# ImNotPrepared/Dynamic3DGaussians

Hardware: AMD Instinct MI355X
Metric: rendered Mpix/s fwd+bwd (1/8 GPU) at 300k Gaussians; PSNR vs ref (higher is better)
Workload: dtype f32

## Files before the change

dynamic3dgaussians_amd/csrc/gs_api.hip:

```cpp
#include <stdarg.h>
#include <stdio.h>
#include <stdlib.h>
#include <string.h>

#include <mutex>
#include <string>
#include <thread>
#include <vector>

#include "../../include/gs_camera_grad.h"
#include "../../include/gs_track.h"
#include "../../include/gs_window.h"
#include "../../include/gsplat_hip.h"
#include "gs_common.h"
#include "gs_kernels.h"
#include "gs_launch.h"

using namespace gs;

namespace {
#define fail gs_set_error

int higher_msb(uint32_t n) {
  uint32_t msb = sizeof(n) * 4, step = msb;
// ... 92 lines not shown
};
thread_local PlanInfo g_plan;

struct HeaderSlot {
  uint32_t* host = nullptr;
  uint32_t* dev = nullptr;
  int device = -1;
};
std::mutex g_hmu;
std::vector<HeaderSlot> g_hfree;

struct HeaderLease {
  HeaderSlot s;
  bool in_flight = false;
  hipStream_t stream = nullptr;
  void launched(hipStream_t s_) {
    in_flight = true;
    stream = s_;
  }
  HeaderLease() {
    int device = 0;
    if (hipGetDevice(&device) != hipSuccess) return;
    {
      std::lock_guard<std::mutex> lk(g_hmu);
      for (size_t i = g_hfree.size(); i-- > 0;) {
        if (g_hfree[i].device != device) continue;
        s = g_hfree[i];
        g_hfree.erase(g_hfree.begin() + (std::ptrdiff_t)i);
        return;
      }
    }
    s.device = device;
    void* h = nullptr;
    if (hipHostMalloc(&h, sizeof(uint32_t) * GS_MAX_CAMS * M_WORDS,
                      hipHostMallocMapped | hipHostMallocCoherent) != hipSuccess)
      return;
    void* d = nullptr;
    if (hipHostGetDevicePointer(&d, h, 0) != hipSuccess) {
      (void)hipHostFree(h);
      s = HeaderSlot{};
      return;
    }
    s.host = static_cast<uint32_t*>(h);
    s.dev = static_cast<uint32_t*>(d);
  }
  ~HeaderLease() {
    if (!s.host) return;
    if (in_flight && hipStreamSynchronize(stream) != hipSuccess) return;
    std::lock_guard<std::mutex> lk(g_hmu);
    g_hfree.push_back(s);
  }
  bool ok() const { return s.host != nullptr; }
};

struct SortPlan {
  int64_t max_len = -1;
  int64_t total = -1;
  SortClasses sc;
  bool hinted = false;
};

SortCover sort_cover(const SortPlan& sp, int64_t tiles) {
  SortCover cv;
  if (sp.max_len < 0 || !sp.sc.valid || !sp.hinted) return cv;
  cv.on = 1;
  cv.q1 = sp.sc.q1;
  cv.p1 = sp.sc.p1;
  cv.p2 = sp.sc.p2;
  cv.mid = sp.max_len > SORT_SMALL;
  cv.lng = sp.max_len > TS_CAP;
  (void)tiles;
  return cv;
}

TileArgs tile_args(int P, int W, int H, void* geom, void* image, const int32_t* walk = nullptr) {
  TileArgs t{};
  t.walk = walk;
  const GeomLayout gl(P);
  const ImgLayout il(W, H);
  t.P = P; t.W = W; t.H = H;
  t.grid_x = (W + TILE - 1) / TILE; t.grid_y = (H + TILE - 1) / TILE;
  t.num_tiles = (int)il.tiles;
  t.rect = at<uint4>(geom, gl.rect);
  t.tiles = at<uint32_t>(geom, gl.tiles);
  t.rec = at<float>(geom, gl.rec);
  t.thist = at<uint32_t>(image, il.thist);
  t.ttotal = at<uint32_t>(image, il.ttotal);
  t.bsum = at<uint32_t>(image, il.bsum);
  t.meta = at<uint32_t>(image, il.meta);
  t.ranges = at<uint2>(image, il.ranges);
  t.order = at<uint4>(image, il.order);
  t.fmax = at<uint32_t>(image, il.fmax);
  return t;
}
}

extern "C" {

int gs_timing_enable(int enable) {
  std::lock_guard<std::mutex> lk(g_tmu);
  for (auto& e : g_events) { g_pool.push_back(e.a); g_pool.push_back(e.b); }
  g_events.clear();
  g_timing = enable != 0;
  return 0;
}

int gs_timing_select(uint32_t stage_mask) {
  std::lock_guard<std::mutex> lk(g_tmu);
  g_timing_mask = stage_mask;
  return 0;
}

int gs_timing_read(double* ms, int64_t* count, int n_kinds) {
  std::lock_guard<std::mutex> lk(g_tmu);
  for (int k = 0; k < n_kinds; ++k) { ms[k] = 0.0; count[k] = 0; }
  for (auto& e : g_events) {
    if (e.kind < 0 || e.kind >= n_kinds) continue;
    hipError_t r = hipEventSynchronize(e.b);
    float t = 0.f;
    if (r == hipSuccess) r = hipEventElapsedTime(&t, e.a, e.b);
    if (r != hipSuccess) return fail((int)r, "timing read: %s", hipGetErrorString(r));
    ms[e.kind] += t;
    count[e.kind] += 1;
  }
  return 0;
}

int gs_version(void) { return GS_ABI_VERSION; }

size_t gs_geom_buffer_bytes(int64_t P) { return GeomLayout(P > 0 ? P : 0).total; }
size_t gs_binning_buffer_bytes(int64_t L) { return BinLayout(L > 0 ? L : 0).total; }
size_t gs_image_buffer_bytes(int32_t W, int32_t H) { return ImgLayout(W, H).total; }
size_t gs_backward_scratch_bytes(int64_t P, int32_t F) { return gs_batch_backward_scratch_bytes(P, F, 1); }


static_assert(GS_WINDOW_MAX_FRAMES == GS_MAX_FRAMES && GS_MAX_FRAMES <= 256, "gs_window.h and CamBatch::frame");
static int make_batch(const gs_camera* cams, int C, int P, int W, int H, CamBatch& cb,
                      const gs_window* win = nullptr) {
  if (C < 1 || C > GS_MAX_CAMS) return fail(-1, "camera batch size %d outside 1..%d", C, GS_MAX_CAMS);
  cb = CamBatch{};
  cb.C = C;
  cb.B = 1;
  if (win) {
    if (int e = gs_check_window(win, C)) return e;
    cb.B = win->B;
    for (int c = 0; c < C; ++c) cb.frame[c] = (uint8_t)win->cam_frame[c];
  }
  cb.geom_stride = (int64_t)GeomLayout(P).total;
  cb.img_stride = (int64_t)ImgLayout(W, H).total;
  cb.view = cams[0].viewmatrix;
  cb.proj = cams[0].projmatrix;
  cb.campos = cams[0].campos;
  for (int c = 0; c < C; ++c) {
    const gs_camera& k = cams[c];
    if (k.image_width != W || k.image_height != H)
      return fail(-1, "camera %d: every camera of a batch has the image size of camera 0", c);
    if (k.viewmatrix != cb.view + 16 * c || k.projmatrix != cb.proj + 16 * c || k.campos != cb.campos + 3 * c)
      return fail(-1, "camera %d: batch camera matrices must be contiguous ([C,16], [C,16], [C,3])", c);
    if (k.background != cams[0].background)
      return fail(-1, "camera %d: the cameras of a batch share one background", c);
    const int gx = (W + TILE - 1) / TILE, gy = (H + TILE - 1) / TILE;
    if (k.tile_x0 == 0 && k.tile_y0 == 0 && k.tile_x1 == 0 && k.tile_y1 == 0) {
      cb.win[c][0] = 0; cb.win[c][1] = 0; cb.win[c][2] = (uint16_t)gx; cb.win[c][3] = (uint16_t)gy;
    } else {
      if (k.tile_x0 < 0 || k.tile_y0 < 0 || k.tile_x0 >= k.tile_x1 || k.tile_y0 >= k.tile_y1 || k.tile_x1 > gx ||
          k.tile_y1 > gy)
        return fail(-1, "camera %d: tile window [%d, %d) x [%d, %d) outside the %d x %d tile grid", c, k.tile_x0,
                    k.tile_x1, k.tile_y0, k.tile_y1, gx, gy);
      cb.win[c][0] = (uint16_t)k.tile_x0; cb.win[c][1] = (uint16_t)k.tile_y0;
      cb.win[c][2] = (uint16_t)k.tile_x1; cb.win[c][3] = (uint16_t)k.tile_y1;
    }
    cb.c_x[c] = k.c_x;
    cb.c_y[c] = k.c_y;
    cb.tanx[c] = k.tan_fovx;
    cb.tany[c] = k.tan_fovy;
  }
  return 0;
}

static int64_t batch_bin_offsets(int C, const int64_t* L, CamBatch* cb) {
  int64_t o = 0;
  for (int c = 0; c < C; ++c) {
    const int64_t l = L ? (L[c] > 0 ? L[c] : 0) : 0;
    if (cb) {
      cb->bin_off[c] = o;
      cb->bin_L[c] = l;
    }
    o += (int64_t)BinLayout(l).total;
  }
  return o;
}

static size_t acc_bytes(int64_t P, int32_t C) {
  return align_up(sizeof(float) * (size_t)ACC_STRIDE * (size_t)(P > 0 ? P : 0) * (C > 0 ? C : 0), 256);
}
static size_t feat_pad_bytes(int64_t P, int32_t F) {
  const int FS = feature_grad_stride(F);
  return FS == F ? 0 : align_up(sizeof(float) * (size_t)FS * (size_t)(P > 0 ? P : 0), 256);
}


static int debug_check_lists(const TileArgs& ta, const CamBatch& cb, const void* binning, const int64_t* L,
                             int64_t P, int64_t tiles, int64_t max_len, hipStream_t s) {
  std::vector<uint32_t> rg((size_t)2 * (tiles > 0 ? tiles : 1)), ids;
  for (int c = 0; c < cb.C; ++c) {
    hipError_t e = hipMemcpyAsync(rg.data(), shift_bytes(ta.ranges, c * cb.img_stride), 8 * (size_t)tiles,
                                  hipMemcpyDeviceToHost, s);
    const int64_t l = L[c] > 0 ? L[c] : 0;
    ids.resize((size_t)(l > 0 ? l : 1));
    if (e == hipSuccess && l > 0)
      e = hipMemcpyAsync(ids.data(), static_cast<const char*>(binning) + cb.bin_off[c], 4 * (size_t)l,
                         hipMemcpyDeviceToHost, s);
    if (e == hipSuccess) e = hipStreamSynchronize(s);
    if (e != hipSuccess) return fail((int)e, "debug readback: %s", hipGetErrorString(e));
    if (int r = gs_check_ranges(rg.data(), tiles, l, max_len)) return r;
    if (int r = gs_check_point_list(ids.data(), l, P)) return r;
  }
  return 0;
}

static int plan_enqueue(const gs_gaussians* g, const gs_camera* cams, int C, int prefiltered, int debug, void* geom,
                        void* image, int32_t* radii, uint32_t* hdr_dev, CamBatch& cb, const gs_window* win,
                        hipStream_t s) {
  const int P = g->P;
  const int W = cams[0].image_width, H = cams[0].image_height;
  if (int e = make_batch(cams, C, P, W, H, cb, win)) return e;
  const GeomLayout gl(P);
  if (debug && g->walk_order && P > 0) {
    std::vector<int32_t> w(P);
    const hipError_t e = hipMemcpyAsync(w.data(), g->walk_order, 4 * (size_t)P, hipMemcpyDeviceToHost, s);
    if (e != hipSuccess || hipStreamSynchronize(s) != hipSuccess)
      return fail((int)e, "walk_order: cannot read it back");
    if (int r = gs_check_walk_order(w.data(), P)) return r;
  }
  const TileArgs ta = tile_args(P, W, H, geom, image, g->walk_order);
  PreprocessArgs a{};
  a.P = P; a.D = g->D; a.M = g->M; a.W = W; a.H = H;
  a.grid_x = ta.grid_x; a.grid_y = ta.grid_y;
  a.prefiltered = prefiltered;
  a.activate = (g->flags & GS_FLAG_ACTIVATE) != 0;
  a.means3D = g->means3D; a.scales = g->scales; a.rotations = g->rotations; a.opacities = g->opacities;
  a.shs = g->shs; a.cov3D_precomp = g->cov3D_precomp; a.colors_precomp = g->colors_precomp;
  a.scale_modifier = g->scale_modifier;
  a.radii = radii;
  a.rec = at<float>(geom, gl.rec);
  a.cov3D = at<float>(geom, gl.cov3D);
  a.clamped = at<uint8_t>(geom, gl.clamped);
  a.tiles = at<uint32_t>(geom, gl.tiles);
  a.rect = at<uint4>(geom, gl.rect);
  a.status = reinterpret_cast<int*>(ta.meta + M_STATUS);
  if (prefiltered)
    for (int c = 0; c < C; ++c) (void)hipMemsetAsync(shift_bytes(a.status, c * cb.img_stride), 0, 4, s);
  {
    StageTimer t(s, GS_STAGE_PREPROCESS);
    launch_preprocess_fwd(a, cb, s);
  }
  if (int e = launch_status("preprocess", debug, s)) return e;
  {
    StageTimer t(s, GS_STAGE_SCAN);
    launch_tile_plan(ta, cb, prefiltered, hdr_dev, s);
  }
  return launch_status("tile plan", debug, s);
}

static int plan_read(const uint32_t (*host)[M_WORDS], int C, int prefiltered, int debug, int64_t tiles,
                     int64_t* num_rendered, int64_t* num_instances, PlanInfo& info) {
  int64_t max_len = 0, total = 0;
  SortClasses sc;
  sc.valid = true;
  sc.q1 = 0x7FFFFFFF;
  for (int c = 0; c < C; ++c) {
    if (debug)
      if (int e = gs_check_plan_header(host[c], tiles)) return e;
    sc.p1 = (int)host[c][M_SORT_P1] > sc.p1 ? (int)host[c][M_SORT_P1] : sc.p1;
    sc.p2 = (int)host[c][M_SORT_P2] > sc.p2 ? (int)host[c][M_SORT_P2] : sc.p2;
    sc.q1 = (int)host[c][M_SORT_Q1] < sc.q1 ? (int)host[c][M_SORT_Q1] : sc.q1;
    if (prefiltered && (host[c][M_STATUS] & 1u))
      return fail(-2, "Point is filtered although prefiltered is set. This shouldn't happen!");
    if (host[c][M_STATUS] & 2u) return fail(-1, "more than 2^32 tile instances");
    num_rendered[c] = host[c][M_LREF];
    if (num_instances) num_instances[c] = host[c][M_L];
    max_len = host[c][M_MAXN] > max_len ? host[c][M_MAXN] : max_len;
    total += host[c][M_L];
  }
  info.C = C;
  info.L = total;
  info.max_len = max_len;
  info.sort = C > 0 ? sc : SortClasses{};
  return 0;
}

static int publish_wait(HeaderLease& hl, int C, hipStream_t s) {
  auto written = [&]() {
    for (int c = 0; c < C; ++c)
      if (__atomic_load_n(&hl.s.host[c * M_WORDS + M_WORDS - 1], __ATOMIC_ACQUIRE) != 0u) return false;
    return true;
  };
  for (uint32_t spin = 1; !written(); ++spin) {
    if ((spin & 4095u) == 0u) {
      const hipError_t q = hipStreamQuery(s);
      if (q == hipSuccess) {
        if (written()) break;
        for (int c = 0; c < C; ++c)
          if (__atomic_load_n(&hl.s.host[c * M_WORDS + M_WORDS - 1], __ATOMIC_ACQUIRE) != 0u)
            return fail(-4, "plan header of camera %d was not written (header path)", c);
      } else if (q != hipErrorNotReady) {
        return fail((int)q, "num_rendered readback: %s", hipGetErrorString(q));
      }
    }
    std::this_thread::yield();
  }
  hl.in_flight = false;
  return 0;
}

static void header_sentinel(HeaderLease& hl, int C) {
  for (int c = 0; c < C; ++c) hl.s.host[c * M_WORDS + M_WORDS - 1] = 0xFFFFFFFFu;
}

static int plan_impl(const gs_gaussians* g, const gs_camera* cams, int C, int prefiltered, int debug, int compat,
                     void* geom, void* image, int32_t* radii, int64_t* num_rendered, int64_t* num_instances,
                     const gs_window* win, hipStream_t s) {
  if (int e = check_gaussians(g, cams, true)) return e;
  if (!num_rendered) return fail(-1, "num_rendered is null");
  for (int c = 0; c < C; ++c) {
    num_rendered[c] = 0;
    if (num_instances) num_instances[c] = 0;
  }
  g_plan = PlanInfo{};
  const int P = g->P;
  if (P == 0) return 0;
// ... 414 lines not shown
}

static_assert(GS_TRACK_MAX_CAMS == GS_MAX_CAMS, "gs_track.h and CamBatch");
int gs_contributors_batch(const gs_camera* cams, int32_t C, int64_t P, int compat, const void* geom,
                          const void* binning, const void* image, const int64_t* L, int32_t K, int32_t* top_id,
                          float* top_w, gs_stream_t stream) {
  if (!cams) return fail(-1, "null argument block");
  if (compat != COMPAT_REFERENCE && compat != COMPAT_FIXED) return fail(-1, "contributors: unknown compat %d", compat);
  const int W = cams[0].image_width, H = cams[0].image_height;
  if (int e = gs_check_contributors(P, C, W, H, K, top_id, top_w)) return e;
  hipStream_t s = (hipStream_t)stream;
  ContribArgs a{};
  a.W = W; a.H = H; a.grid_x = (W + TILE - 1) / TILE; a.num_tiles = a.grid_x * ((H + TILE - 1) / TILE); a.K = K;
  a.top_id = top_id; a.top_w = top_w;
  CamBatch cb{};
  cb.C = C;
  int64_t total = 0;
  if (P > 0 && L)
    for (int c = 0; c < C; ++c) total += L[c] > 0 ? L[c] : 0;
  const bool walk = P > 0 && total > 0 && a.num_tiles > 0;
  if (walk) {
    if (!geom || !binning || !image) return fail(-1, "contributors: state buffers are required");
    if (int e = make_batch(cams, C, (int)P, W, H, cb)) return e;
    batch_bin_offsets(C, L, &cb);
    a.order = at<uint4>(image, ImgLayout(W, H).order);
    a.point_list = static_cast<const uint32_t*>(binning);
    a.rec = at<float>(geom, GeomLayout(P).rec);
  }
  launch_contributors(a, cb, walk, s);
  return launch_status("contributors", 0, s);
}

int gs_track_project(const gs_camera* cams, int32_t C, int64_t P, int32_t T, const float* means3D, const int32_t* ids,
                     int64_t N, float* uv, float* depth, uint8_t* inside, gs_stream_t stream) {
  if (!cams) return fail(-1, "null argument block");
  if (int e = gs_check_track_project(P, T, C, N, ids, uv, depth, inside)) return e;
  if ((int64_t)T * C * N == 0) return 0;
  const int W = cams[0].image_width, H = cams[0].image_height;
  if (W <= 0 || H <= 0) return fail(-1, "image size must be positive (got %dx%d)", W, H);
  if (P > 0 && (!means3D || !cams[0].viewmatrix || !cams[0].projmatrix))
    return fail(-1, "track project: means3D and the camera matrices are required");
  CamBatch cb;
  if (int e = make_batch(cams, C, (int)P, W, H, cb)) return e;
  TrackProjectArgs a{};
  a.P = (int)P; a.T = T; a.W = W; a.H = H; a.N = N;
  a.means3D = means3D; a.ids = ids; a.uv = uv; a.depth = depth; a.inside = inside;
  launch_track_project(a, cb, (hipStream_t)stream);
  return launch_status("track project", 0, (hipStream_t)stream);
}

int gs_mark_visible(int64_t P, const float* means3D, const float* viewmatrix, const float* projmatrix,
                    uint8_t* present, gs_stream_t stream) {
  (void)projmatrix;
  if (P < 0) return fail(-1, "P must be >= 0");
  if (P == 0) return 0;
  if (!means3D || !viewmatrix || !present) return fail(-1, "null argument");
  hipStream_t s = (hipStream_t)stream;
  launch_mark_visible((int)P, means3D, viewmatrix, present, s);
  return launch_status("markVisible", 0, s);
}

int gs_debug_export(int64_t P, int32_t W, int32_t H, const void* geom, const void* binning, const void* image,
                    int64_t L, float* means2D, float* depths, float* conic_opacity, float* rgb,
                    uint32_t* tiles_touched, uint32_t* point_list, uint32_t* ranges, uint32_t* n_contrib,
                    gs_stream_t stream) {
  hipStream_t s = (hipStream_t)stream;
  const GeomLayout gl(P);
  const BinLayout bl(L);
  const ImgLayout il(W, H);
  const float* rec = at<float>(geom, gl.rec);
  hipError_t e = hipSuccess;
  auto cp2d = [&](float* dst, int cols, int first) {
    if (dst && P > 0 && e == hipSuccess)
      e = hipMemcpy2DAsync(dst, sizeof(float) * cols, rec + first, sizeof(float) * REC, sizeof(float) * cols,
                           (size_t)P, hipMemcpyDeviceToDevice, s);
  };
  cp2d(means2D, 2, R_X);
  cp2d(depths, 1, R_DEPTH);
  if (conic_opacity && P > 0 && e == hipSuccess)
    e = hipMemcpy2DAsync(conic_opacity, sizeof(float) * 4, rec + R_CA, sizeof(float) * REC, sizeof(float) * 4,
                         (size_t)P, hipMemcpyDeviceToDevice, s);
  cp2d(rgb, 3, R_R);
  if (tiles_touched && P > 0 && e == hipSuccess)
    e = hipMemcpyAsync(tiles_touched, at<uint32_t>(geom, gl.tiles), 4 * P, hipMemcpyDeviceToDevice, s);
  if (point_list && L > 0 && e == hipSuccess)
    e = hipMemcpyAsync(point_list, at<uint32_t>(binning, bl.plist), 4 * L,
                       hipMemcpyDeviceToDevice, s);
  const int64_t tiles = (int64_t)((W + TILE - 1) / TILE) * ((H + TILE - 1) / TILE);
  if (ranges && e == hipSuccess)
    e = hipMemcpyAsync(ranges, at<uint32_t>(image, il.ranges), 8 * tiles, hipMemcpyDeviceToDevice, s);
  if (n_contrib && e == hipSuccess)
    e = hipMemcpyAsync(n_contrib, at<uint32_t>(image, il.n_contrib), 4 * (size_t)W * H, hipMemcpyDeviceToDevice, s);
  if (e != hipSuccess) return fail((int)e, "debug export: %s", hipGetErrorString(e));
  return 0;
}

int gs_test_wave_reduce(int n_comp, const float* in, float* out, gs_stream_t stream) {
  if (n_comp < 1 || n_comp > 64) return fail(-1, "n_comp must be in [1, 64]");
  launch_test_wave_reduce(n_comp, in, out, (hipStream_t)stream);
  return launch_status("wave reduce test", 1, (hipStream_t)stream);
}

}
```

dynamic3dgaussians_amd/csrc/gs_common.h:

```cpp
#pragma once

#include <hip/hip_runtime.h>
#include <stdint.h>

#include <type_traits>

#include "gs_meta.h"

namespace gs {

constexpr int TILE = 16;
constexpr int TILE_PIX = TILE * TILE;
constexpr int WAVE = 64;
constexpr int STRIP_W = 8, STRIP_H = 8;
constexpr int STRIPS_X = TILE / STRIP_W;
__host__ __device__ inline int strip_x0(int tx, int s) { return tx * TILE + (s % STRIPS_X) * STRIP_W; }
__host__ __device__ inline int strip_y0(int ty, int s) { return ty * TILE + (s / STRIPS_X) * STRIP_H; }

constexpr int REC = 16;
enum RecField {
  R_X = 0, R_Y = 1,
  R_CA = 2, R_CB = 3, R_CC = 4,
  R_OP = 5,
  R_R = 6, R_G = 7, R_B = 8,
  R_DEPTH = 9,
  R_EX = 10, R_EY = 11,
  R_RAD = 12,
  R_TQ = 13,
};

enum AccField {
  A_MX = 0, A_MY = 1, A_CA = 2, A_CB = 3, A_CC = 4, A_OP = 5,
  A_R = 6, A_G = 7, A_B = 8, A_DEPTH = 9, A_FEAT = 10,
};
constexpr int ACC_STRIDE = 16;

constexpr int COMPAT_REFERENCE = 0;
constexpr int COMPAT_FIXED = 1;

__host__ __device__ inline size_t align_up(size_t x, size_t a) { return (x + a - 1) / a * a; }

constexpr int SORT_THREADS = 256;
__host__ __device__ inline int sort_rounds(int64_t n) {
  int64_t r = (n + (int64_t)SORT_THREADS * 2048 - 1) / ((int64_t)SORT_THREADS * 2048);
  return (int)(r < 1 ? 1 : (r > 16 ? 16 : r));
}
__host__ __device__ inline int64_t sort_blocks(int64_t n) {
  const int64_t tile = (int64_t)SORT_THREADS * sort_rounds(n);
  return (n + tile - 1) / tile;
}
constexpr int TB_BLOCKS = 128;
constexpr int TB_THREADS = 1024;
constexpr int TB_BINS = 16384;
constexpr int SORT_SMALL = 1024;
constexpr int TS_CAP = 4096;
constexpr int TS_CAP_LONG = 9600;
constexpr int TS_WIDE_MEAN = 1024;

struct GeomLayout {
  size_t rec, cov3D, clamped, tiles, rect, total;
  __host__ __device__ GeomLayout(int64_t P) {
    size_t o = 0;
    rec = o;       o = align_up(o + sizeof(float) * REC * P, 256);
    cov3D = o;     o = align_up(o + sizeof(float) * 6 * P, 256);
    clamped = o;   o = align_up(o + P, 256);
    tiles = o;     o = align_up(o + sizeof(uint32_t) * P, 256);
    rect = o;      o = align_up(o + sizeof(uint32_t) * 4 * P, 256);
    total = o;
  }
};

struct BinLayout {
  size_t plist, keys, keys2, total;
  __host__ __device__ BinLayout(int64_t L) {
    size_t o = 0;
    plist = o; o = align_up(o + sizeof(uint32_t) * L, 256);
    keys = o;  o = align_up(o + sizeof(uint64_t) * L, 256);
    keys2 = o; o = align_up(o + sizeof(uint64_t) * L, 256);
    total = o;
  }
};

struct SortLayout {
  size_t keys1, vals1, hist, rowtot, total;
  __host__ __device__ SortLayout(int64_t n) {
    const int64_t nblk = sort_blocks(n);
    size_t o = 0;
    keys1 = o; o = align_up(o + sizeof(uint64_t) * n, 256);
    vals1 = o; o = align_up(o + sizeof(uint32_t) * n, 256);
    hist = o;  o = align_up(o + sizeof(uint32_t) * 256 * (nblk > 0 ? nblk : 1), 256);
    rowtot = o; o = align_up(o + sizeof(uint32_t) * 256, 256);
    total = o;
  }
};

struct ImgLayout {
  size_t ranges, n_contrib, thist, ttotal, bsum, meta, order, smax, fmax, total;
  int64_t tiles;
  __host__ __device__ ImgLayout(int W, int H) {
    tiles = (int64_t)((W + TILE - 1) / TILE) * ((H + TILE - 1) / TILE);
    const int64_t t = tiles > 0 ? tiles : 1;
    size_t o = 0;
    ranges = o;    o = align_up(o + sizeof(uint32_t) * 2 * t, 256);
    n_contrib = o; o = align_up(o + sizeof(uint32_t) * (int64_t)W * H, 256);
    thist = o;     o = align_up(o + sizeof(uint32_t) * TB_BLOCKS * t, 256);
    ttotal = o;    o = align_up(o + sizeof(uint32_t) * t, 256);
    bsum = o;      o = align_up(o + sizeof(uint32_t) * TB_BLOCKS, 256);
    meta = o;      o = align_up(o + sizeof(uint32_t) * M_WORDS, 256);
    order = o;     o = align_up(o + sizeof(uint32_t) * 4 * t, 256);
    smax = o;      o = align_up(o + sizeof(uint32_t) * 4 * t, 256);
    fmax = o;      o = align_up(o + sizeof(uint32_t) * 64, 256);
    total = o;
  }
};

constexpr int GS_MAX_CAMS = 64;
constexpr int GS_MAX_FRAMES = 64;
struct CamBatch {
  int C;
  int64_t geom_stride;
  int64_t img_stride;
  const float* view;
  const float* proj;
  const float* campos;
  float c_x[GS_MAX_CAMS], c_y[GS_MAX_CAMS], tanx[GS_MAX_CAMS], tany[GS_MAX_CAMS];
  int64_t bin_off[GS_MAX_CAMS];
  int64_t bin_L[GS_MAX_CAMS];
  uint16_t win[GS_MAX_CAMS][4];
  uint8_t frame[GS_MAX_CAMS];
  int B;
};
static_assert(sizeof(CamBatch) <= 4096 - 512, "CamBatch outgrew the kernel-argument budget");
__host__ __device__ inline size_t mean_offset(const CamBatch& cb, int c, int g) {
  return 3 * ((size_t)g * cb.B + cb.frame[c]);
}
__host__ __device__ inline bool in_window(const CamBatch& cb, int c, int tx, int ty) {
  return tx >= cb.win[c][0] && tx < cb.win[c][2] && ty >= cb.win[c][1] && ty < cb.win[c][3];
}
template <class T>
__host__ __device__ inline T* shift_bytes(T* p, int64_t bytes) {
  return p ? reinterpret_cast<T*>(reinterpret_cast<char*>(const_cast<typename std::remove_const<T>::type*>(p)) + bytes)
           : p;
}


__device__ inline bool rect_culled(float mx, float my, float a, float b, float c, float tq, float sx0,
                                   float sx1, float sy0, float sy1) {
  const float xlo = mx - sx1, xhi = mx - sx0;
  const float ylo = my - sy1, yhi = my - sy0;
// ... 112 lines not shown
```

dynamic3dgaussians_amd/csrc/gs_kernels.h:

```cpp
#pragma once

#include <hip/hip_ext.h>
#include <hip/hip_runtime.h>
#include <stdint.h>

#include "gs_common.h"

namespace gs {

struct PreprocessArgs {
  int P, D, M, W, H, grid_x, grid_y, prefiltered;
  int activate;
  const float* means3D;
  const float* scales;
  const float* rotations;
  const float* opacities;
  const float* shs;
  const float* cov3D_precomp;
  const float* colors_precomp;
  const float* view;
  const float* proj;
  const float* campos;
  float scale_modifier, c_x, c_y, tan_fovx, tan_fovy, focal_x, focal_y;
  int* radii;
  float* rec;
  float* cov3D;
  uint8_t* clamped;
  uint32_t* tiles;
  uint4* rect;
  int* status;
};

struct PreprocessBwdArgs {
  int P, D, M, F, W, H, compat;
  int accumulate;
  int activate;
  const float* opacities;
  const float* means3D;
  const int* radii;
  const float* shs;
  const uint8_t* clamped;
  const float* scales;
  const float* rotations;
  const float* cov3D;
  const float* cov3D_precomp;
  const float* view;
  const float* proj;
  const float* campos;
  float scale_modifier, c_x, c_y, tan_fovx, tan_fovy, focal_x, focal_y;
  const float* rec;
  const float* acc;
  const float* grad_mask;
  float* st_accum;
  float* st_denom;
  float* st_maxrad;
  float* dmeans2D;
  float* dcolors;
  float* dsemantic;
  float* dopacity;
  float* dmeans3D;
  float* dcov3D;
  float* dsh;
  float* dscales;
  float* drot;
};

struct RenderArgs {
  int W, H, grid_x, num_tiles, F, compat, P;
  const uint4* order;
  const uint2* ranges;
  const uint32_t* point_list;
  const float* rec;
  const float* feats;
  uint32_t* smax;
  const float* bg;
  float* out_color;
  float* out_feature;
  float* out_depth;
  float* out_alpha;
  uint32_t* n_contrib;
  const uint32_t* fmax;
  float4* zero;
  int64_t zero_n;
};

__host__ __device__ constexpr int feature_grad_stride(int F) {
  return (F < 16 || F % 16 == 0) ? F : (F + 15) / 16 * 16;
}
void launch_feature_grad_rows(const float* pad, float* out, int64_t P, int F, int accumulate, hipStream_t s);
void launch_feature_absmax(const float* feats, int64_t P, int F, uint32_t* out, hipStream_t s);

struct RenderBwdArgs {
  int W, H, grid_x, num_tiles, F, compat, P;
  const uint4* order;
  const uint2* ranges;
  const uint32_t* point_list;
  const float* rec;
  const float* feats;
  const float* bg;
  const uint32_t* smax;
  const float* alphas;
  const uint32_t* n_contrib;
  const float* dL_dpix;
  const float* dL_dfeat;
  const float* dL_ddepth;
  const float* dL_dalpha;
  float* acc;
  float* dsem;
};

struct LaunchEvents {
  hipEvent_t start = nullptr, stop = nullptr;
};
LaunchEvents& launch_events();
template <class K, class... A>
inline void timed_launch(K kernel, dim3 grid, dim3 block, uint32_t lds, hipStream_t s, A... args) {
  LaunchEvents& e = launch_events();
  if (e.start) {
    const LaunchEvents ev = e;
    e = LaunchEvents{};
    hipExtLaunchKernelGGL(kernel, grid, block, lds, s, ev.start, ev.stop, 0u, args...);
  } else {
    hipLaunchKernelGGL(kernel, grid, block, lds, s, args...);
  }
}

void launch_preprocess_fwd(const PreprocessArgs& a, const CamBatch& cb, hipStream_t s);
void launch_preprocess_bwd(const PreprocessBwdArgs& a, const CamBatch& cb, hipStream_t s);
void launch_mark_visible(int P, const float* means3D, const float* view, uint8_t* present, hipStream_t s);

struct CameraGradArgs {
  int P, D, M, W, H;
  const float* means3D;
  const int* radii;
  const float* shs;
  const uint8_t* clamped;
  const float* cov3D;
  const float* cov3D_precomp;
  const float* rec;
  const float* acc;
  double* records;
  float* dview;
  float* dproj;
  float* dcampos;
};
void launch_camera_grad(const CameraGradArgs& a, const CamBatch& cb, hipStream_t s);

struct ContribArgs {
  int W, H, grid_x, num_tiles, K;
  const uint4* order;
  const uint32_t* point_list;
  const float* rec;
  int32_t* top_id;
  float* top_w;
};
void launch_contributors(const ContribArgs& a, const CamBatch& cb, bool walk, hipStream_t s);
struct TrackProjectArgs {
  int P, T, W, H;
  int64_t N;
  const float* means3D;
  const int32_t* ids;
  float* uv;
  float* depth;
  uint8_t* inside;
};
void launch_track_project(const TrackProjectArgs& a, const CamBatch& cb, hipStream_t s);

int launch_radix_sort(int64_t n, uint64_t* keys0, uint32_t* vals0, uint64_t* keys1, uint32_t* vals1,
                      uint32_t* hist, uint32_t* rowtot, int end_bit, hipStream_t s);

struct TileArgs {
  int P, W, H, grid_x, grid_y, num_tiles;
  const uint4* rect;
  const uint32_t* tiles;
  const float* rec;
  uint32_t* thist;
  uint32_t* ttotal;
  uint32_t* bsum;
  uint32_t* meta;
  uint2* ranges;
  uint4* order;
  uint32_t* fmax;
  uint64_t* keys;
  uint64_t* keys2;
  uint32_t* plist;
  void* binning;
  const int32_t* walk;
};
__host__ __device__ inline TileArgs cam_tile_args(const TileArgs& a0, const CamBatch& cb, int c) {
  TileArgs a = a0;
  const int64_t go = c * cb.geom_stride, io = c * cb.img_stride;
  a.rect = shift_bytes(a0.rect, go);
  a.tiles = shift_bytes(a0.tiles, go);
  a.rec = shift_bytes(a0.rec, go);
  a.thist = shift_bytes(a0.thist, io);
  a.ttotal = shift_bytes(a0.ttotal, io);
  a.bsum = shift_bytes(a0.bsum, io);
  a.meta = shift_bytes(a0.meta, io);
  a.ranges = shift_bytes(a0.ranges, io);
  a.order = shift_bytes(a0.order, io);
  if (a0.binning) {
    char* b = static_cast<char*>(a0.binning) + cb.bin_off[c];
    const BinLayout bl(cb.bin_L[c]);
    a.plist = reinterpret_cast<uint32_t*>(b + bl.plist);
    a.keys = reinterpret_cast<uint64_t*>(b + bl.keys);
    a.keys2 = reinterpret_cast<uint64_t*>(b + bl.keys2);
  }
  return a;
}
void launch_tile_plan(const TileArgs& a, const CamBatch& cb, int prefiltered, uint32_t* hdr_host, hipStream_t s);
void launch_tile_bucket(const TileArgs& a, const CamBatch& cb, hipStream_t s);
struct SortCover {
  int on = 0;
  int q1 = 0, p1 = 0, p2 = 0;
  int mid = 0, lng = 0;
};
void launch_tile_order(const TileArgs& a, const CamBatch& cb, const SortCover& cv, hipStream_t s);
struct SortClasses {
  bool valid = false;
  int p1 = 0, q1 = 0, p2 = 0;
};
void launch_tile_sort(const TileArgs& a, const CamBatch& cb, int64_t max_len, int64_t L, const SortClasses& sc,
                      hipStream_t s);

__host__ __device__ inline RenderArgs cam_render_args(const RenderArgs& a0, const CamBatch& cb, int c) {
  RenderArgs a = a0;
  const int64_t go = c * cb.geom_stride, io = c * cb.img_stride, hw = (int64_t)a0.W * a0.H;
  a.order = shift_bytes(a0.order, io);
  a.ranges = shift_bytes(a0.ranges, io);
  a.smax = shift_bytes(a0.smax, io);
  a.n_contrib = shift_bytes(a0.n_contrib, io);
  a.rec = shift_bytes(a0.rec, go);
  a.point_list = shift_bytes(a0.point_list, cb.bin_off[c]);
  a.out_color = a0.out_color ? a0.out_color + c * 3 * hw : nullptr;
  a.out_feature = a0.out_feature ? a0.out_feature + c * a0.F * hw : nullptr;
  a.out_depth = a0.out_depth ? a0.out_depth + c * hw : nullptr;
  a.out_alpha = a0.out_alpha ? a0.out_alpha + c * hw : nullptr;
  return a;
}
__host__ __device__ inline RenderBwdArgs cam_render_bwd_args(const RenderBwdArgs& a0, const CamBatch& cb, int c) {
  RenderBwdArgs a = a0;
  const int64_t go = c * cb.geom_stride, io = c * cb.img_stride, hw = (int64_t)a0.W * a0.H;
  a.order = shift_bytes(a0.order, io);
  a.ranges = shift_bytes(a0.ranges, io);
  a.smax = shift_bytes(a0.smax, io);
  a.n_contrib = shift_bytes(a0.n_contrib, io);
  a.rec = shift_bytes(a0.rec, go);
  a.point_list = shift_bytes(a0.point_list, cb.bin_off[c]);
  a.alphas = a0.alphas ? a0.alphas + c * hw : nullptr;
  a.dL_dpix = a0.dL_dpix ? a0.dL_dpix + c * 3 * hw : nullptr;
  a.dL_dfeat = a0.dL_dfeat ? a0.dL_dfeat + c * a0.F * hw : nullptr;
  a.dL_ddepth = a0.dL_ddepth ? a0.dL_ddepth + c * hw : nullptr;
  a.dL_dalpha = a0.dL_dalpha ? a0.dL_dalpha + c * hw : nullptr;
  a.acc = a0.acc + (size_t)c * a0.P * ACC_STRIDE;
  return a;
}
bool launch_render_fwd(const RenderArgs& a, const CamBatch& cb, hipStream_t s);
bool launch_render_bwd(const RenderBwdArgs& a, const CamBatch& cb, hipStream_t s);

void launch_test_wave_reduce(int n, const float* in, float* out, hipStream_t s);

}
```

dynamic3dgaussians_amd/csrc/gs_preprocess.hip:

```cpp
#include "gs_activate.h"
#include "gs_common.h"
#include "gs_kernels.h"
#include "gs_project.h"

namespace gs {

__device__ inline void tile_rect(float px, float py, int r, int gx, int gy, int2& rmin, int2& rmax) {
  int a;
  a = (int)((px - (float)r) / (float)TILE); a = a > 0 ? a : 0; rmin.x = a < gx ? a : gx;
  a = (int)((py - (float)r) / (float)TILE); a = a > 0 ? a : 0; rmin.y = a < gy ? a : gy;
  a = (int)((((px + (float)r) + (float)TILE) - 1.0f) / (float)TILE); a = a > 0 ? a : 0; rmax.x = a < gx ? a : gx;
  a = (int)((((py + (float)r) + (float)TILE) - 1.0f) / (float)TILE); a = a > 0 ? a : 0; rmax.y = a < gy ? a : gy;
}

__device__ inline void quat_cols(float4 q, float rc[3][3]) {
  const float r = q.x, x = q.y, y = q.z, z = q.w;
  rc[0][0] = 1.f - 2.f * (y * y + z * z); rc[0][1] = 2.f * (x * y - r * z); rc[0][2] = 2.f * (x * z + r * y);
  rc[1][0] = 2.f * (x * y + r * z); rc[1][1] = 1.f - 2.f * (x * x + z * z); rc[1][2] = 2.f * (y * z - r * x);
  rc[2][0] = 2.f * (x * z - r * y); rc[2][1] = 2.f * (y * z + r * x); rc[2][2] = 1.f - 2.f * (x * x + y * y);
}

__device__ inline void alpha_extent(float ca, float cb, float cc, float op, float& ex, float& ey, float& tq) {
  const float thr = 1.0f / 255.0f;
  if (!(op >= thr)) { ex = -INFINITY; ey = -INFINITY; tq = -INFINITY; return; }
  const double a = ca, b = cb, c = cc;
  const double det = a * c - b * b;
  const double tr = a + c;
  if (!(a > 0.0 && c > 0.0 && det > 0.0)) { ex = INFINITY; ey = INFINITY; tq = INFINITY; return; }
  const double disc = sqrt(fmax(tr * tr - 4.0 * det, 0.0));
  const double lmin = 0.5 * (tr - disc), lmax = 0.5 * (tr + disc);
  const double cond = lmin > 0.0 ? lmax / lmin : 1e30;
  if (!(cond < 5.0e5)) { ex = INFINITY; ey = INFINITY; tq = INFINITY; return; }
  const double tau = 2.0 * (double)logf(op * 255.0f);
  const double taup = tau * (1.02 + 32.0 * 6.0e-8 * cond) + 1e-3;
  ex = (float)(sqrt(taup * c / det) + 0.01);
  ey = (float)(sqrt(taup * a / det) + 0.01);
  tq = (float)(taup * 1.0001 + 1e-4);
}

__device__ inline void sh_fwd(int deg, int M, V3 p, V3 cp, const float* __restrict__ shs, int g,
                              float rgb[3], uint8_t& clampbits) {
  float dx = p.x - cp.x, dy = p.y - cp.y, dz = p.z - cp.z;
  const float len = sqrtf(dx * dx + dy * dy + dz * dz);
  const float x = dx / len, y = dy / len, z = dz / len;
  const float* sh = shs + (size_t)g * M * 3;
  clampbits = 0;
#pragma unroll
  for (int ch = 0; ch < 3; ++ch) {
#define S(i) sh[3 * (i) + ch]
    float res = SH_C0 * S(0);
    if (deg > 0) {
      res = res - SH_C1 * y * S(1) + SH_C1 * z * S(2) - SH_C1 * x * S(3);
      if (deg > 1) {
        const float xx = x * x, yy = y * y, zz = z * z, xy = x * y, yz = y * z, xz = x * z;
        res = res + SH_C2_0 * xy * S(4) + SH_C2_1 * yz * S(5) + SH_C2_2 * (2.0f * zz - xx - yy) * S(6) +
              SH_C2_3 * xz * S(7) + SH_C2_4 * (xx - yy) * S(8);
        if (deg > 2) {
          res = res + SH_C3_0 * y * (3.0f * xx - yy) * S(9) + SH_C3_1 * xy * z * S(10) +
                SH_C3_2 * y * (4.0f * zz - xx - yy) * S(11) +
                SH_C3_3 * z * (2.0f * zz - 3.0f * xx - 3.0f * yy) * S(12) +
                SH_C3_4 * x * (4.0f * zz - xx - yy) * S(13) + SH_C3_5 * z * (xx - yy) * S(14) +
                SH_C3_6 * x * (xx - 3.0f * yy) * S(15);
        }
      }
    }
#undef S
    res += 0.5f;
    if (res < 0.0f) clampbits |= (uint8_t)(1u << ch);
    rgb[ch] = res > 0.0f ? res : 0.0f;
  }
}

__device__ inline float act_sigmoid(float x) { return 1.0f / (1.0f + expf(-x)); }
__device__ inline float4 rotation_of(const float* __restrict__ rotations, int g, int activate) {
  const float4 q = reinterpret_cast<const float4*>(rotations)[g];
  return activate ? act_normalize(q) : q;
}
__device__ inline V3 scale_of(const float* __restrict__ scales, int g, int activate) {
  const V3 s = ld3(scales + 3 * g);
  return activate ? V3{expf(s.x), expf(s.y), expf(s.z)} : s;
}


__device__ inline PreprocessArgs cam_args(const PreprocessArgs& a0, const CamBatch& cb, int c) {
  PreprocessArgs a = a0;
  a.view = cb.view + 16 * c;
  a.proj = cb.proj + 16 * c;
  a.campos = cb.campos + 3 * c;
  a.c_x = cb.c_x[c];
  a.c_y = cb.c_y[c];
  a.tan_fovx = cb.tanx[c];
  a.tan_fovy = cb.tany[c];
  a.focal_y = (float)a.H / (2.0f * a.tan_fovy);
  a.focal_x = (float)a.W / (2.0f * a.tan_fovx);
  const int64_t go = c * cb.geom_stride;
  a.radii = a0.radii + (size_t)c * a0.P;
  a.rec = shift_bytes(a0.rec, go);
  a.cov3D = shift_bytes(a0.cov3D, go);
  a.clamped = shift_bytes(a0.clamped, go);
  a.tiles = shift_bytes(a0.tiles, go);
  a.rect = shift_bytes(a0.rect, go);
  a.status = shift_bytes(a0.status, c * cb.img_stride);
  return a;
}

__global__ __launch_bounds__(256) void preprocess_fwd_kernel(PreprocessArgs a0, CamBatch batch) {
  const int cam = blockIdx.y, g = blockIdx.x * 256 + threadIdx.x;
  if (g >= a0.P) return;
  const PreprocessArgs a = cam_args(a0, batch, cam);
  auto culled = [&]() {
    a.radii[g] = 0;
    a.tiles[g] = 0;
    a.rect[g] = make_uint4(0u, 0u, 0u, 0u);
  };
  const V3 p = ld3(a.means3D + mean_offset(batch, cam, g));
  float c3[6];
  if (a.cov3D_precomp) {
#pragma unroll
    for (int i = 0; i < 6; ++i) c3[i] = a.cov3D_precomp[6 * g + i];
  } else {
    float rc[3][3];
    const float4 q = rotation_of(a.rotations, g, a.activate);
    quat_cols(q, rc);
    const V3 s = scale_of(a.scales, g, a.activate);
    const float sx = a.scale_modifier * s.x, sy = a.scale_modifier * s.y, sz = a.scale_modifier * s.z;
    float m[3][3];
#pragma unroll
    for (int c = 0; c < 3; ++c) { m[c][0] = sx * rc[c][0]; m[c][1] = sy * rc[c][1]; m[c][2] = sz * rc[c][2]; }
#define DOT3(i, j) (m[i][0] * m[j][0] + m[i][1] * m[j][1] + m[i][2] * m[j][2])
    c3[0] = DOT3(0, 0); c3[1] = DOT3(0, 1); c3[2] = DOT3(0, 2);
    c3[3] = DOT3(1, 1); c3[4] = DOT3(1, 2); c3[5] = DOT3(2, 2);
#undef DOT3
    if (cam == 0) {
#pragma unroll
      for (int i = 0; i < 6; ++i) a.cov3D[6 * g + i] = c3[i];
    }
  }
  const V3 pv = xf43(a.view, p);
  if (pv.z <= 0.0f) {
    if (a.prefiltered) atomicOr(a.status, 1);
    culled();
    return;
  }
  const float4 ph = xf44(a.proj, p);
  const float pw = 1.0f / (ph.w + 0.0000001f);
  const float ppx = ph.x * pw, ppy = ph.y * pw;
  Ewa e;
  ewa_setup(p, a.view, a.W, a.H, a.c_x, a.c_y, a.focal_x, a.focal_y, a.tan_fovx, a.tan_fovy, e);
  float cov[3];
  ewa_cov2d(e, c3, cov);
  const float det = cov[0] * cov[2] - cov[1] * cov[1];
  if (det == 0.0f) {
    culled();
    return;
  }
  const float det_inv = 1.f / det;
  const float ca = cov[2] * det_inv, cb = -cov[1] * det_inv, cc = cov[0] * det_inv;
  const float mid = 0.5f * (cov[0] + cov[2]);
  const float l1 = mid + sqrtf(fmaxf(0.1f, mid * mid - det));
  const float l2 = mid - sqrtf(fmaxf(0.1f, mid * mid - det));
  const float rad = ceilf(3.f * sqrtf(fmaxf(l1, l2)));
  const float px = ndc_to_pix(ppx, a.W), py = ndc_to_pix(ppy, a.H);
  int2 rmin, rmax;
  tile_rect(px, py, (int)rad, a.grid_x, a.grid_y, rmin, rmax);
  if ((rmax.x - rmin.x) * (rmax.y - rmin.y) == 0) {
    culled();
    return;
  }

  float rgb[3];
  if (a.colors_precomp) {
    rgb[0] = a.colors_precomp[3 * g]; rgb[1] = a.colors_precomp[3 * g + 1]; rgb[2] = a.colors_precomp[3 * g + 2];
  } else {
    uint8_t cl;
    sh_fwd(a.D, a.M, p, ld3(a.campos), a.shs, g, rgb, cl);
    a.clamped[g] = cl;
  }
  const float op = a.activate ? act_sigmoid(a.opacities[g]) : a.opacities[g];
  float ex, ey, tq;
  alpha_extent(ca, cb, cc, op, ex, ey, tq);
  float4* rec = reinterpret_cast<float4*>(a.rec + (size_t)REC * g);
  rec[0] = make_float4(px, py, ca, cb);
  rec[1] = make_float4(cc, op, rgb[0], rgb[1]);
  rec[2] = make_float4(rgb[2], pv.z, ex, ey);
  rec[3] = make_float4((float)rad, tq, 0.f, 0.f);
  a.radii[g] = (int)rad;
  a.tiles[g] = (uint32_t)((rmax.y - rmin.y) * (rmax.x - rmin.x));
  const float fx0 = fminf(fmaxf(ceilf((px - ex - (TILE - 1)) / TILE), (float)rmin.x), (float)rmax.x);
  const float fx1 = fminf(fmaxf(floorf((px + ex) / TILE) + 1.f, (float)rmin.x), (float)rmax.x);
  const float fy0 = fminf(fmaxf(ceilf((py - ey - (TILE - 1)) / TILE), (float)rmin.y), (float)rmax.y);
  const float fy1 = fminf(fmaxf(floorf((py + ey) / TILE) + 1.f, (float)rmin.y), (float)rmax.y);
  const uint16_t* win = batch.win[cam];
  const int bx0 = max((int)fx0, (int)win[0]), by0 = max((int)fy0, (int)win[1]);
  const int bx1 = max(min((int)fx1, (int)win[2]), bx0), by1 = max(min((int)fy1, (int)win[3]), by0);
  a.rect[g] = make_uint4((uint32_t)bx0 | ((uint32_t)by0 << 16), (uint32_t)bx1 | ((uint32_t)by1 << 16),
                         __float_as_uint(pv.z), (uint32_t)((rmax.y - rmin.y) * (rmax.x - rmin.x)));
}

void launch_preprocess_fwd(const PreprocessArgs& a, const CamBatch& cb, hipStream_t s) {
  if (a.P <= 0) return;
  hipLaunchKernelGGL(preprocess_fwd_kernel, dim3((a.P + 255) / 256, cb.C), dim3(256), 0, s, a, cb);
}

__global__ __launch_bounds__(256) void mark_visible_kernel(int P, const float* __restrict__ means3D,
                                                           const float* __restrict__ view,
                                                           uint8_t* __restrict__ present) {
  const int g = blockIdx.x * 256 + threadIdx.x;
  if (g >= P) return;
  const V3 pv = xf43(view, ld3(means3D + 3 * g));
  present[g] = !(pv.z <= 0.0f);
}

void launch_mark_visible(int P, const float* means3D, const float* view, uint8_t* present, hipStream_t s) {
  if (P <= 0) return;
  hipLaunchKernelGGL(mark_visible_kernel, dim3((P + 255) / 256), dim3(256), 0, s, P, means3D, view, present);
}


__device__ inline void gput(float* p, float v, int accumulate) { *p = accumulate ? *p + v : v; }

__device__ inline void sh_bwd(int deg, int M, V3 mean, V3 cp, const float* __restrict__ shs, int g,
                              uint8_t clampbits, const float dcolor[3], float* __restrict__ dsh_out,
                              float dmean[3], float mk, int accumulate) {
  const float dox = mean.x - cp.x, doy = mean.y - cp.y, doz = mean.z - cp.z;
  const float len = sqrtf(dox * dox + doy * doy + doz * doz);
  const float x = dox / len, y = doy / len, z = doz / len;
  const float* sh = shs + (size_t)g * M * 3;
  float* ds = dsh_out + (size_t)g * M * 3;
  float dRGB[3];
#pragma unroll
  for (int ch = 0; ch < 3; ++ch) dRGB[ch] = dcolor[ch] * (((clampbits >> ch) & 1) ? 0.0f : 1.0f);
  float ddx[3] = {0, 0, 0}, ddy[3] = {0, 0, 0}, ddz[3] = {0, 0, 0};
  const int ncoef = (deg + 1) * (deg + 1);
  if (!accumulate)
    for (int i = ncoef; i < M; ++i) { ds[3 * i] = 0.f * mk; ds[3 * i + 1] = 0.f * mk; ds[3 * i + 2] = 0.f * mk; }
#pragma unroll
  for (int ch = 0; ch < 3; ++ch) {
#define S(i) sh[3 * (i) + ch]
#define WR(i, v) gput(ds + 3 * (i) + ch, ((v) * dRGB[ch]) * mk, accumulate)
    WR(0, SH_C0);
    if (deg > 0) {
      WR(1, -SH_C1 * y); WR(2, SH_C1 * z); WR(3, -SH_C1 * x);
      ddx[ch] = -SH_C1 * S(3); ddy[ch] = -SH_C1 * S(1); ddz[ch] = SH_C1 * S(2);
      if (deg > 1) {
        const float xx = x * x, yy = y * y, zz = z * z, xy = x * y, yz = y * z, xz = x * z;
        WR(4, SH_C2_0 * xy); WR(5, SH_C2_1 * yz); WR(6, SH_C2_2 * (2.f * zz - xx - yy));
        WR(7, SH_C2_3 * xz); WR(8, SH_C2_4 * (xx - yy));
        ddx[ch] += SH_C2_0 * y * S(4) + SH_C2_2 * 2.f * -x * S(6) + SH_C2_3 * z * S(7) + SH_C2_4 * 2.f * x * S(8);
        ddy[ch] += SH_C2_0 * x * S(4) + SH_C2_1 * z * S(5) + SH_C2_2 * 2.f * -y * S(6) + SH_C2_4 * 2.f * -y * S(8);
        ddz[ch] += SH_C2_1 * y * S(5) + SH_C2_2 * 2.f * 2.f * z * S(6) + SH_C2_3 * x * S(7);
        if (deg > 2) {
          WR(9, SH_C3_0 * y * (3.f * xx - yy)); WR(10, SH_C3_1 * xy * z);
          WR(11, SH_C3_2 * y * (4.f * zz - xx - yy)); WR(12, SH_C3_3 * z * (2.f * zz - 3.f * xx - 3.f * yy));
          WR(13, SH_C3_4 * x * (4.f * zz - xx - yy)); WR(14, SH_C3_5 * z * (xx - yy));
          WR(15, SH_C3_6 * x * (xx - 3.f * yy));
          ddx[ch] += (SH_C3_0 * S(9) * 3.f * 2.f * xy + SH_C3_1 * S(10) * yz + SH_C3_2 * S(11) * -2.f * xy +
                      SH_C3_3 * S(12) * -3.f * 2.f * xz + SH_C3_4 * S(13) * (-3.f * xx + 4.f * zz - yy) +
                      SH_C3_5 * S(14) * 2.f * xz + SH_C3_6 * S(15) * 3.f * (xx - yy));
          ddy[ch] += (SH_C3_0 * S(9) * 3.f * (xx - yy) + SH_C3_1 * S(10) * xz +
                      SH_C3_2 * S(11) * (-3.f * yy + 4.f * zz - xx) + SH_C3_3 * S(12) * -3.f * 2.f * yz +
                      SH_C3_4 * S(13) * -2.f * xy + SH_C3_5 * S(14) * -2.f * yz + SH_C3_6 * S(15) * -3.f * 2.f * xy);
          ddz[ch] += (SH_C3_1 * S(10) * xy + SH_C3_2 * S(11) * 4.f * 2.f * yz +
                      SH_C3_3 * S(12) * 3.f * (2.f * zz - xx - yy) + SH_C3_4 * S(13) * 4.f * 2.f * xz +
                      SH_C3_5 * S(14) * (xx - yy));
        }
      }
    }
#undef S
#undef WR
  }
  const float dd0 = ddx[0] * dRGB[0] + ddx[1] * dRGB[1] + ddx[2] * dRGB[2];
  const float dd1 = ddy[0] * dRGB[0] + ddy[1] * dRGB[1] + ddy[2] * dRGB[2];
  const float dd2 = ddz[0] * dRGB[0] + ddz[1] * dRGB[1] + ddz[2] * dRGB[2];
  const float s2 = dox * dox + doy * doy + doz * doz;
  const float inv = 1.0f / sqrtf(s2 * s2 * s2);
  dmean[0] += ((s2 - dox * dox) * dd0 - doy * dox * dd1 - doz * dox * dd2) * inv;
  dmean[1] += (-dox * doy * dd0 + (s2 - doy * doy) * dd1 - doz * doy * dd2) * inv;
  dmean[2] += (-dox * doz * dd0 - doy * doz * dd1 + (s2 - doz * doz) * dd2) * inv;
}

__device__ inline void cov3d_bwd(V3 scale, float mod, float4 rot, const float d[6], float dscale[3],
                                 float drot[4]) {
  float rc[3][3];
  quat_cols(rot, rc);
// ... 252 lines not shown
```

Measured before the change: 2227.

## Batch four cameras per preprocess thread and drop redundant tiles buffer

The forward preprocess kernel now handles up to four cameras per thread. The camera-independent 3D covariance, opacity activation and precomputed colors are computed once and reused across those cameras, and means are reloaded only when the frame changes. The separate per-Gaussian tiles array is removed because the count is already stored in rect.w, and the debug export now copies it from there with a strided copy. This cuts redundant math and global writes at the cost of fewer blocks in the grid's y dimension and more per-thread work and registers.

```diff
diff --git a/dynamic3dgaussians_amd/csrc/gs_api.hip b/dynamic3dgaussians_amd/csrc/gs_api.hip
--- a/dynamic3dgaussians_amd/csrc/gs_api.hip
+++ b/dynamic3dgaussians_amd/csrc/gs_api.hip
@@ -198,7 +198,6 @@
   t.grid_x = (W + TILE - 1) / TILE; t.grid_y = (H + TILE - 1) / TILE;
   t.num_tiles = (int)il.tiles;
   t.rect = at<uint4>(geom, gl.rect);
-  t.tiles = at<uint32_t>(geom, gl.tiles);
   t.rec = at<float>(geom, gl.rec);
   t.thist = at<uint32_t>(image, il.thist);
   t.ttotal = at<uint32_t>(image, il.ttotal);
@@ -362,7 +361,6 @@
   a.rec = at<float>(geom, gl.rec);
   a.cov3D = at<float>(geom, gl.cov3D);
   a.clamped = at<uint8_t>(geom, gl.clamped);
-  a.tiles = at<uint32_t>(geom, gl.tiles);
   a.rect = at<uint4>(geom, gl.rect);
   a.status = reinterpret_cast<int*>(ta.meta + M_STATUS);
   if (prefiltered)
@@ -943,7 +941,8 @@
                          (size_t)P, hipMemcpyDeviceToDevice, s);
   cp2d(rgb, 3, R_R);
   if (tiles_touched && P > 0 && e == hipSuccess)
-    e = hipMemcpyAsync(tiles_touched, at<uint32_t>(geom, gl.tiles), 4 * P, hipMemcpyDeviceToDevice, s);
+    e = hipMemcpy2DAsync(tiles_touched, sizeof(uint32_t), at<uint32_t>(geom, gl.rect) + 3, sizeof(uint4),
+                         sizeof(uint32_t), (size_t)P, hipMemcpyDeviceToDevice, s);
   if (point_list && L > 0 && e == hipSuccess)
     e = hipMemcpyAsync(point_list, at<uint32_t>(binning, bl.plist), 4 * L,
                        hipMemcpyDeviceToDevice, s);
diff --git a/dynamic3dgaussians_amd/csrc/gs_common.h b/dynamic3dgaussians_amd/csrc/gs_common.h
--- a/dynamic3dgaussians_amd/csrc/gs_common.h
+++ b/dynamic3dgaussians_amd/csrc/gs_common.h
@@ -58,13 +58,12 @@
 constexpr int TS_WIDE_MEAN = 1024;
 
 struct GeomLayout {
-  size_t rec, cov3D, clamped, tiles, rect, total;
+  size_t rec, cov3D, clamped, rect, total;
   __host__ __device__ GeomLayout(int64_t P) {
     size_t o = 0;
     rec = o;       o = align_up(o + sizeof(float) * REC * P, 256);
     cov3D = o;     o = align_up(o + sizeof(float) * 6 * P, 256);
     clamped = o;   o = align_up(o + P, 256);
-    tiles = o;     o = align_up(o + sizeof(uint32_t) * P, 256);
     rect = o;      o = align_up(o + sizeof(uint32_t) * 4 * P, 256);
     total = o;
   }
diff --git a/dynamic3dgaussians_amd/csrc/gs_kernels.h b/dynamic3dgaussians_amd/csrc/gs_kernels.h
--- a/dynamic3dgaussians_amd/csrc/gs_kernels.h
+++ b/dynamic3dgaussians_amd/csrc/gs_kernels.h
@@ -26,7 +26,6 @@
   float* rec;
   float* cov3D;
   uint8_t* clamped;
-  uint32_t* tiles;
   uint4* rect;
   int* status;
 };
@@ -172,7 +171,6 @@
 struct TileArgs {
   int P, W, H, grid_x, grid_y, num_tiles;
   const uint4* rect;
-  const uint32_t* tiles;
   const float* rec;
   uint32_t* thist;
   uint32_t* ttotal;
@@ -191,7 +189,6 @@
   TileArgs a = a0;
   const int64_t go = c * cb.geom_stride, io = c * cb.img_stride;
   a.rect = shift_bytes(a0.rect, go);
-  a.tiles = shift_bytes(a0.tiles, go);
   a.rec = shift_bytes(a0.rec, go);
   a.thist = shift_bytes(a0.thist, io);
   a.ttotal = shift_bytes(a0.ttotal, io);
diff --git a/dynamic3dgaussians_amd/csrc/gs_preprocess.hip b/dynamic3dgaussians_amd/csrc/gs_preprocess.hip
--- a/dynamic3dgaussians_amd/csrc/gs_preprocess.hip
+++ b/dynamic3dgaussians_amd/csrc/gs_preprocess.hip
@@ -98,44 +98,23 @@
   a.rec = shift_bytes(a0.rec, go);
   a.cov3D = shift_bytes(a0.cov3D, go);
   a.clamped = shift_bytes(a0.clamped, go);
-  a.tiles = shift_bytes(a0.tiles, go);
   a.rect = shift_bytes(a0.rect, go);
   a.status = shift_bytes(a0.status, c * cb.img_stride);
   return a;
 }
 
-__global__ __launch_bounds__(256) void preprocess_fwd_kernel(PreprocessArgs a0, CamBatch batch) {
-  const int cam = blockIdx.y, g = blockIdx.x * 256 + threadIdx.x;
-  if (g >= a0.P) return;
-  const PreprocessArgs a = cam_args(a0, batch, cam);
+struct GaussianShared {
+  float c3[6];
+  float op;
+  float rgb[3];
+};
+
+__device__ inline void project_camera(const PreprocessArgs& a, const CamBatch& batch, int cam, int g, V3 p,
+                                      const GaussianShared& sh) {
   auto culled = [&]() {
     a.radii[g] = 0;
-    a.tiles[g] = 0;
     a.rect[g] = make_uint4(0u, 0u, 0u, 0u);
   };
-  const V3 p = ld3(a.means3D + mean_offset(batch, cam, g));
-  float c3[6];
-  if (a.cov3D_precomp) {
-#pragma unroll
-    for (int i = 0; i < 6; ++i) c3[i] = a.cov3D_precomp[6 * g + i];
-  } else {
-    float rc[3][3];
-    const float4 q = rotation_of(a.rotations, g, a.activate);
-    quat_cols(q, rc);
-    const V3 s = scale_of(a.scales, g, a.activate);
-    const float sx = a.scale_modifier * s.x, sy = a.scale_modifier * s.y, sz = a.scale_modifier * s.z;
-    float m[3][3];
-#pragma unroll
-    for (int c = 0; c < 3; ++c) { m[c][0] = sx * rc[c][0]; m[c][1] = sy * rc[c][1]; m[c][2] = sz * rc[c][2]; }
-#define DOT3(i, j) (m[i][0] * m[j][0] + m[i][1] * m[j][1] + m[i][2] * m[j][2])
-    c3[0] = DOT3(0, 0); c3[1] = DOT3(0, 1); c3[2] = DOT3(0, 2);
-    c3[3] = DOT3(1, 1); c3[4] = DOT3(1, 2); c3[5] = DOT3(2, 2);
-#undef DOT3
-    if (cam == 0) {
-#pragma unroll
-      for (int i = 0; i < 6; ++i) a.cov3D[6 * g + i] = c3[i];
-    }
-  }
   const V3 pv = xf43(a.view, p);
   if (pv.z <= 0.0f) {
     if (a.prefiltered) atomicOr(a.status, 1);
@@ -148,7 +127,7 @@
   Ewa e;
   ewa_setup(p, a.view, a.W, a.H, a.c_x, a.c_y, a.focal_x, a.focal_y, a.tan_fovx, a.tan_fovy, e);
   float cov[3];
-  ewa_cov2d(e, c3, cov);
+  ewa_cov2d(e, sh.c3, cov);
   const float det = cov[0] * cov[2] - cov[1] * cov[1];
   if (det == 0.0f) {
     culled();
@@ -170,13 +149,13 @@
 
   float rgb[3];
   if (a.colors_precomp) {
-    rgb[0] = a.colors_precomp[3 * g]; rgb[1] = a.colors_precomp[3 * g + 1]; rgb[2] = a.colors_precomp[3 * g + 2];
+    rgb[0] = sh.rgb[0]; rgb[1] = sh.rgb[1]; rgb[2] = sh.rgb[2];
   } else {
     uint8_t cl;
     sh_fwd(a.D, a.M, p, ld3(a.campos), a.shs, g, rgb, cl);
     a.clamped[g] = cl;
   }
-  const float op = a.activate ? act_sigmoid(a.opacities[g]) : a.opacities[g];
+  const float op = sh.op;
   float ex, ey, tq;
   alpha_extent(ca, cb, cc, op, ex, ey, tq);
   float4* rec = reinterpret_cast<float4*>(a.rec + (size_t)REC * g);
@@ -185,7 +164,6 @@
   rec[2] = make_float4(rgb[2], pv.z, ex, ey);
   rec[3] = make_float4((float)rad, tq, 0.f, 0.f);
   a.radii[g] = (int)rad;
-  a.tiles[g] = (uint32_t)((rmax.y - rmin.y) * (rmax.x - rmin.x));
   const float fx0 = fminf(fmaxf(ceilf((px - ex - (TILE - 1)) / TILE), (float)rmin.x), (float)rmax.x);
   const float fx1 = fminf(fmaxf(floorf((px + ex) / TILE) + 1.f, (float)rmin.x), (float)rmax.x);
   const float fy0 = fminf(fmaxf(ceilf((py - ey - (TILE - 1)) / TILE), (float)rmin.y), (float)rmax.y);
@@ -197,9 +175,52 @@
                          __float_as_uint(pv.z), (uint32_t)((rmax.y - rmin.y) * (rmax.x - rmin.x)));
 }
 
+constexpr int PF_CAMS = 4;
+
+__global__ __launch_bounds__(256) void preprocess_fwd_kernel(PreprocessArgs a0, CamBatch batch) {
+  const int cam0 = blockIdx.y * PF_CAMS, g = blockIdx.x * 256 + threadIdx.x;
+  if (g >= a0.P) return;
+  GaussianShared sh;
+  if (a0.cov3D_precomp) {
+#pragma unroll
+    for (int i = 0; i < 6; ++i) sh.c3[i] = a0.cov3D_precomp[6 * g + i];
+  } else {
+    float rc[3][3];
+    const float4 q = rotation_of(a0.rotations, g, a0.activate);
+    quat_cols(q, rc);
+    const V3 s = scale_of(a0.scales, g, a0.activate);
+    const float sx = a0.scale_modifier * s.x, sy = a0.scale_modifier * s.y, sz = a0.scale_modifier * s.z;
+    float m[3][3];
+#pragma unroll
+    for (int c = 0; c < 3; ++c) { m[c][0] = sx * rc[c][0]; m[c][1] = sy * rc[c][1]; m[c][2] = sz * rc[c][2]; }
+#define DOT3(i, j) (m[i][0] * m[j][0] + m[i][1] * m[j][1] + m[i][2] * m[j][2])
+    sh.c3[0] = DOT3(0, 0); sh.c3[1] = DOT3(0, 1); sh.c3[2] = DOT3(0, 2);
+    sh.c3[3] = DOT3(1, 1); sh.c3[4] = DOT3(1, 2); sh.c3[5] = DOT3(2, 2);
+#undef DOT3
+    if (cam0 == 0) {
+#pragma unroll
+      for (int i = 0; i < 6; ++i) a0.cov3D[6 * g + i] = sh.c3[i];
+    }
+  }
+  sh.op = a0.activate ? act_sigmoid(a0.opacities[g]) : a0.opacities[g];
+  if (a0.colors_precomp) {
+    sh.rgb[0] = a0.colors_precomp[3 * g]; sh.rgb[1] = a0.colors_precomp[3 * g + 1];
+    sh.rgb[2] = a0.colors_precomp[3 * g + 2];
+  }
+  V3 p = ld3(a0.means3D + mean_offset(batch, cam0, g));
+#pragma unroll
+  for (int k = 0; k < PF_CAMS; ++k) {
+    const int cam = cam0 + k;
+    if (cam >= batch.C) break;
+    if (k > 0 && batch.frame[cam] != batch.frame[cam - 1]) p = ld3(a0.means3D + mean_offset(batch, cam, g));
+    project_camera(cam_args(a0, batch, cam), batch, cam, g, p, sh);
+  }
+}
+
 void launch_preprocess_fwd(const PreprocessArgs& a, const CamBatch& cb, hipStream_t s) {
   if (a.P <= 0) return;
-  hipLaunchKernelGGL(preprocess_fwd_kernel, dim3((a.P + 255) / 256, cb.C), dim3(256), 0, s, a, cb);
+  hipLaunchKernelGGL(preprocess_fwd_kernel, dim3((a.P + 255) / 256, (cb.C + PF_CAMS - 1) / PF_CAMS), dim3(256), 0, s,
+                     a, cb);
 }
 
 __global__ __launch_bounds__(256) void mark_visible_kernel(int P, const float* __restrict__ means3D,
```

Result: no change. 2226 (-0.1%).
